# nschejtman/deepLoopCloser

Measured on AMD Instinct MI355X. Metric: query-frames/sec vs N-keyframe DB + top-k recall@1, higher is better.
Workload: dtype bf16; 1 GPU; 1000000 x 4096 bf16 keyframe DB, Q=256, top-20 cosine match, 1 GPU(s); db_rows=1000000, dim=4096, k=20, rows_per_gpu=1000000, pipelined=False, crowded=False

## Files before the change

deeploopcloser_amd/csrc/cosine_topk.hip:

```cpp
#include "dlc_internal.h"

#include <algorithm>

namespace {

constexpr int BM = 256;
constexpr int BNQ = 256;
constexpr int BK = 64;
constexpr int NTHREADS = 512;
constexpr int TILE_BYTES = 256 * BK * 2;
constexpr int A_TILE = TILE_BYTES;
constexpr int B_TILE = TILE_BYTES;
#ifndef DLC_A_STAGES
#define DLC_A_STAGES 2
#endif
constexpr int A_STAGES = DLC_A_STAGES;
constexpr int B_RING = A_STAGES * A_TILE;
constexpr int LDS_BYTES = A_STAGES * A_TILE + 2 * B_TILE;
#ifndef DLC_STAGGER_SLEEP
#define DLC_STAGGER_SLEEP 15
#endif
#ifndef DLC_STAGGER_PHASES
#define DLC_STAGGER_PHASES 32
#endif
// ... 3 lines not shown
constexpr int GROUPS_PER_HALF = HALF / GROUP;
constexpr int SLACK = 4;

template <typename Tag> struct Mfma16;
template <> struct Mfma16<dlc_bf16_tag> {
    static __device__ __forceinline__ f32x4_t run(u32x4_t a, u32x4_t b, f32x4_t c) {
        return __builtin_amdgcn_mfma_f32_16x16x32_bf16(__builtin_bit_cast(bf16x8_t, a),
                                                       __builtin_bit_cast(bf16x8_t, b), c, 0, 0, 0);
    }
    static __device__ __forceinline__ float to_f32(unsigned short h) { return dlc_bf16_bits_to_f32(h); }
};
template <> struct Mfma16<dlc_f16_tag> {
    static __device__ __forceinline__ f32x4_t run(u32x4_t a, u32x4_t b, f32x4_t c) {
        return __builtin_amdgcn_mfma_f32_16x16x32_f16(__builtin_bit_cast(f16x8_t, a),
                                                      __builtin_bit_cast(f16x8_t, b), c, 0, 0, 0);
    }
    static __device__ __forceinline__ float to_f32(unsigned short h) { return dlc_f16_bits_to_f32(h); }
};

typedef const __attribute__((address_space(1))) void* gptr_t;
typedef __attribute__((address_space(3))) void* lptr_t;

__device__ __forceinline__ void glds16(const char* g, char* l) {
    __builtin_amdgcn_global_load_lds((gptr_t)g, (lptr_t)l, 16, 0, 0);
}

__device__ __forceinline__ int swz_a(int r) { return ((r >> 1) & 1) | (((r >> 4) & 3) << 1); }
__device__ __forceinline__ int swz_b(int r) { return (r >> 1) & 7; }

struct GemmArgs {
    const char* Q;
    const char* DB;
    long long ldq_b;
    long long lddb_b;
    int q;
    long long n;
    int nk;
    float* gmax;
    long long ldg;
    float* tmax;
    long long ldt;
    long long ng;
    long long nh;
    float* S;
    long long lds;
    int stagger_mult;
    int stagger_phases;
    int nqb;
    long long ntiles;
    int nsplit;
    int kchunk;
    float* P;
    long long ldp;
};

constexpr int GEMM_GROUPS = 0;
constexpr int GEMM_DENSE = 1;
constexpr int GEMM_PARTIAL = 2;

constexpr int HALF_BYTES = 128 * 128;

#ifndef DLC_A_CACHE_POLICY
#define DLC_A_CACHE_POLICY " nt"
#endif
#define DLC_DMA4_BODY(POLICY)                                \
    asm volatile(                                            \
        "s_nop 4\n\t"                                        \
        "s_mov_b32 %0, m0\n\t"                               \
        "s_mov_b32 m0, %6\n\t"                               \
        "s_nop 0\n\t"                                        \
        "global_load_lds_dwordx4 %1, %5" POLICY "\n\t"       \
        "s_add_u32 m0, %6, 0x400\n\t"                        \
        "s_nop 0\n\t"                                        \
        "global_load_lds_dwordx4 %2, %5" POLICY "\n\t"       \
        "s_add_u32 m0, %6, 0x800\n\t"                        \
        "s_nop 0\n\t"                                        \
        "global_load_lds_dwordx4 %3, %5" POLICY "\n\t"       \
        "s_add_u32 m0, %6, 0xc00\n\t"                        \
        "s_nop 0\n\t"                                        \
        "global_load_lds_dwordx4 %4, %5" POLICY "\n\t"       \
        "s_mov_b32 m0, %0"                                   \
        : "=&s"(keep)                                        \
        : "v"(voff[0]), "v"(voff[1]), "v"(voff[2]), "v"(voff[3]), "s"(sbase), "s"(lds0) \
        : "memory", "scc")
__device__ __forceinline__ void dma4(const unsigned (&voff)[4], const char* sbase, unsigned lds0) {
    unsigned keep;
    DLC_DMA4_BODY("");
}
__device__ __forceinline__ void dma4_stream(const unsigned (&voff)[4], const char* sbase, unsigned lds0) {
    unsigned keep;
    DLC_DMA4_BODY(DLC_A_CACHE_POLICY);
}

#define DLC_WAIT_VMCNT(n) asm volatile("s_waitcnt vmcnt(" #n ")" ::: "memory")
#define DLC_WAIT_LGKM0() asm volatile("s_waitcnt lgkmcnt(0)" ::: "memory")
__device__ __forceinline__ void wg_barrier() {
    asm volatile("" ::: "memory");
    __builtin_amdgcn_s_barrier();
    asm volatile("" ::: "memory");
}

template <typename Tag, int MODE, bool MASKQ>
__global__ __launch_bounds__(NTHREADS, 2) void score_gemm_kernel(GemmArgs p) {
    extern __shared__ __attribute__((aligned(16))) char smem[];
    const int tid = threadIdx.x;
    const int lane = tid & 63;
    const int wid = __builtin_amdgcn_readfirstlane(tid >> 6);
// ... 147 lines not shown
#undef DLC_READ_A
#undef DLC_READ_B
#undef DLC_MFMA
#undef DLC_RELEASE

    const int lg = lane >> 4;
    if constexpr (MODE == GEMM_PARTIAL) {
        float* part = p.P + (long long)chunk * p.q * p.ldp;
#pragma unroll
        for (int c = 0; c < 4; ++c) {
            const int qidx = qblk * BNQ + wc * 64 + c * 16 + i;
            if (qidx >= p.q) continue;
#pragma unroll
            for (int t = 0; t < 8; ++t) {
                const long long row0 = tile * BM + wr * 128 + (t >> 2) * 64 + 16 * lg + 4 * (t & 3);
                *(f32x4_t*)(part + (long long)qidx * p.ldp + row0) = acc[t][c];
            }
        }
    } else if constexpr (MODE == GEMM_DENSE) {
#pragma unroll
        for (int c = 0; c < 4; ++c) {
            const int qidx = qblk * BNQ + wc * 64 + c * 16 + i;
            if (qidx >= p.q) continue;
#pragma unroll
            for (int t = 0; t < 8; ++t) {
                const long long row0 = tile * BM + wr * 128 + (t >> 2) * 64 + 16 * lg + 4 * (t & 3);
#pragma unroll
                for (int r = 0; r < 4; ++r)
                    if (row0 + r < p.n) p.S[(long long)qidx * p.lds + row0 + r] = acc[t][c][r];
            }
        }
    } else {
#pragma unroll
        for (int c = 0; c < 4; ++c) {
            const int qidx = qblk * BNQ + wc * 64 + c * 16 + i;
            float hm[2];
#pragma unroll
            for (int th = 0; th < 2; ++th) {
                float m0 = acc[th * 4][c][0], m1 = acc[th * 4 + 2][c][0];
#pragma unroll
                for (int tt = 0; tt < 2; ++tt)
#pragma unroll
                    for (int r = 0; r < 4; ++r) {
                        m0 = fmaxf(m0, acc[th * 4 + tt][c][r]);
                        m1 = fmaxf(m1, acc[th * 4 + 2 + tt][c][r]);
                    }
                hm[th] = fmaxf(m0, m1);
                const long long g = tile * (BM / GROUP) + wr * 16 + th * 8 + lg * 2;
                if (qidx < p.q) {
                    float* dst = p.gmax + (long long)qidx * p.ldg + g;
                    if (g + 1 < p.ng) *(float2*)dst = make_float2(m0, m1);
                    else if (g < p.ng) dst[0] = m0;
                }
            }
            float h = fmaxf(hm[0], hm[1]);
            h = fmaxf(h, __shfl_xor(h, 16));
            h = fmaxf(h, __shfl_xor(h, 32));
            const long long ht = tile * 2 + wr;
            if (lg == 0 && qidx < p.q && ht < p.nh) p.tmax[(long long)qidx * p.ldt + ht] = h;
        }
    }
}

template <typename Tag> struct Dot2;
template <> struct Dot2<dlc_bf16_tag> {
    typedef __attribute__((ext_vector_type(2))) __bf16 v2_t;
    static __device__ __forceinline__ float run(unsigned a, unsigned b, float c) {
        return __builtin_amdgcn_fdot2_f32_bf16(__builtin_bit_cast(v2_t, a), __builtin_bit_cast(v2_t, b), c, false);
    }
};
template <> struct Dot2<dlc_f16_tag> {
    typedef __attribute__((ext_vector_type(2))) _Float16 v2_t;
    static __device__ __forceinline__ float run(unsigned a, unsigned b, float c) {
        return __builtin_amdgcn_fdot2(__builtin_bit_cast(v2_t, a), __builtin_bit_cast(v2_t, b), c, false);
    }
};

constexpr int GEMV_MAX_Q = 4;
constexpr int GEMV_MAX_LDS = 64 * 1024;

template <typename Tag, int QB>
__global__ __launch_bounds__(256) void score_gemv_kernel(GemmArgs p) {
    extern __shared__ __attribute__((aligned(16))) char smem[];
    __shared__ float wmax[4][QB];
    const int tid = threadIdx.x, lane = tid & 63, w = tid >> 6;
    const long long half = blockIdx.x;
    const int d_bytes = p.nk * 128;
    for (int off = tid * 16; off < QB * d_bytes; off += 256 * 16) {
        const int qi = off / d_bytes, within = off - qi * d_bytes;
        uint4 v = make_uint4(0, 0, 0, 0);
        if (qi < p.q) v = *(const uint4*)(p.Q + (long long)qi * p.ldq_b + within);
        *(uint4*)(smem + off) = v;
    }
    __syncthreads();
    float hmax[QB];
#pragma unroll
    for (int qq = 0; qq < QB; ++qq) hmax[qq] = -INFINITY;
    for (int gi = 0; gi < 4; ++gi) {
        const long long g = half * GROUPS_PER_HALF + w * 4 + gi;
        const char* rows[GROUP];
#pragma unroll
        for (int r = 0; r < GROUP; ++r) {
            long long rr = g * GROUP + r;
            if (rr > p.n - 1) rr = p.n - 1;
            rows[r] = p.DB + rr * p.lddb_b;
        }
// ... 28 lines not shown
                float v = acc[qq][r];
#pragma unroll
                for (int o = 32; o > 0; o >>= 1) v += __shfl_xor(v, o);
                m = fmaxf(m, v);
            }
            hmax[qq] = fmaxf(hmax[qq], m);
            if (lane == 0 && qq < p.q && g < p.ng) p.gmax[(long long)qq * p.ldg + g] = m;
        }
    }
    if (lane == 0) {
#pragma unroll
        for (int qq = 0; qq < QB; ++qq) wmax[w][qq] = hmax[qq];
    }
    __syncthreads();
    if (tid < QB && tid < p.q && half < p.nh)
        p.tmax[(long long)tid * p.ldt + half] = fmaxf(fmaxf(wmax[0][tid], wmax[1][tid]), fmaxf(wmax[2][tid], wmax[3][tid]));
}

__device__ __forceinline__ unsigned f32_key(float x) {
    unsigned u = __float_as_uint(x);
    return (u & 0x80000000u) ? ~u : (u | 0x80000000u);
}
__device__ __forceinline__ float key_f32(unsigned k) {
    return __uint_as_float((k & 0x80000000u) ? (k ^ 0x80000000u) : ~k);
}
__device__ __forceinline__ unsigned long long pack_key(float score, unsigned id) {
    return ((unsigned long long)f32_key(score) << 32) | (unsigned long long)(~id);
}
__device__ __forceinline__ unsigned key_id(unsigned long long key) { return ~(unsigned)key; }

constexpr long long KEY64_EMPTY = (long long)0x8000000000000000ull;
__device__ __forceinline__ long long f64_key(double s) {
    const double x = s * 1099511627776.0;
    if (!(x > -4.0e18)) return KEY64_EMPTY + 1;
    if (x > 4.0e18) return 0x7fffffffffffffffll;
    return __double2ll_rn(x);
}

__device__ __forceinline__ unsigned wave_max_u32(unsigned v) {
#define DLC_DPP_MAX(ctrl, rmask) \
    v = max(v, (unsigned)__builtin_amdgcn_update_dpp((int)v, (int)v, ctrl, rmask, 0xf, false))
    DLC_DPP_MAX(0x111, 0xf);
    DLC_DPP_MAX(0x112, 0xf);
    DLC_DPP_MAX(0x114, 0xf);
    DLC_DPP_MAX(0x118, 0xf);
    DLC_DPP_MAX(0x142, 0xa);
    DLC_DPP_MAX(0x143, 0xc);
#undef DLC_DPP_MAX
    return (unsigned)__builtin_amdgcn_readlane((int)v, 63);
}

constexpr int FIN_THREADS = 512;
__host__ __device__ inline size_t fin_lds_fixed(int kg) {
    return (size_t)kg * (GROUPS_PER_HALF * 8 + GROUP * (8 + 8 + 4)) + (size_t)(kg + 1) * 8 + 64;
}

__device__ __forceinline__ void rank_select(const unsigned long long* keys, int m, int k, int* out, bool plus_one = false) {
    const int lim = plus_one ? k + 1 : k;
    for (int e = threadIdx.x; e < m; e += blockDim.x) {
        const unsigned long long ke = keys[e];
        if (ke == 0ull) continue;
        int rank = 0;
#pragma unroll 8
        for (int j = 0; j < m; ++j) rank += keys[j] > ke ? 1 : 0;
        if (rank < lim) out[rank] = e;
    }
}
template <typename Id>
__device__ __forceinline__ void rank_select64(const long long* keys, const Id* ids, int m, int k, int* out) {
    for (int e = threadIdx.x; e < m; e += blockDim.x) {
        const long long ke = keys[e];
        if (ke == KEY64_EMPTY) continue;
        const Id ie = ids[e];
        int rank = 0;
#pragma unroll 4
        for (int j = 0; j < m; ++j) {
            const long long kj = keys[j];
            rank += (kj > ke || (kj == ke && kj != KEY64_EMPTY && ids[j] < ie)) ? 1 : 0;
        }
        if (rank < k) out[rank] = e;
    }
}

template <typename Tag, int RS_UNROLL>
__device__ __forceinline__ void rescore8_f64(const char* qrow, const char* const (&rows)[GROUP], int d, int lane,
                                             double (&acc)[GROUP]) {
#pragma unroll
    for (int r = 0; r < GROUP; ++r) acc[r] = 0.0;
    for (int d0 = lane * 8; d0 < d; d0 += 512 * RS_UNROLL) {
        uint4 qv[RS_UNROLL], rv[RS_UNROLL][GROUP];
#pragma unroll
        for (int u = 0; u < RS_UNROLL; ++u) {
            const int dd = d0 + u * 512;
            const bool ok = dd < d;
            qv[u] = ok ? *(const uint4*)(qrow + (long long)dd * 2) : make_uint4(0, 0, 0, 0);
#pragma unroll
            for (int r = 0; r < GROUP; ++r)
                rv[u][r] = ok ? *(const uint4*)(rows[r] + (long long)dd * 2) : make_uint4(0, 0, 0, 0);
        }
#pragma unroll
        for (int u = 0; u < RS_UNROLL; ++u) {
            const unsigned qw[4] = {qv[u].x, qv[u].y, qv[u].z, qv[u].w};
            double qd[8];
#pragma unroll
            for (int e = 0; e < 4; ++e) {
                qd[2 * e] = (double)Mfma16<Tag>::to_f32((unsigned short)(qw[e] & 0xffffu));
                qd[2 * e + 1] = (double)Mfma16<Tag>::to_f32((unsigned short)(qw[e] >> 16));
// ... 48 lines not shown
#pragma unroll
                for (int e = 0; e < 4; ++e) {
                    acc[r] = fma(qd[2 * e], (double)Mfma16<Tag>::to_f32((unsigned short)(w4[e] & 0xffffu)), acc[r]);
                    acc[r] = fma(qd[2 * e + 1], (double)Mfma16<Tag>::to_f32((unsigned short)(w4[e] >> 16)), acc[r]);
                }
            }
        }
    }
#pragma unroll
    for (int r = 0; r < R; ++r) {
        double v = acc[r];
#pragma unroll
        for (int o = 32; o > 0; o >>= 1) v += __shfl_xor(v, o);
        acc[r] = v;
    }
}
template <typename Tag>
__device__ __forceinline__ double rescore1_f64(const char* qrow, const char* row, int d, int lane) {
    const char* const rows[1] = {row};
    double acc[1];
    rescore_rows_f64<Tag, 1, 4>(qrow, rows, d, lane, acc);
    return acc[0];
}

__device__ __forceinline__ double scaled_tau(double tau, const float* __restrict__ tau_scale, int qi) {
    return tau_scale ? tau * (double)tau_scale[qi] : tau;
}

enum { FIN_FUSED = 0, FIN_GROUPS = 1, FIN_RESCORE = 2 };
struct FinishArgs {
    float* tmax; long long ldt; int nh; int tv_in_lds;
    const float* gmax; long long ldg; long long ng;
    int kg;
    const char* Q; long long ldq_b; const char* DB; long long lddb_b;
    long long n; int d; int k; long long row_offset;
    float* out_s;
    double* out_s64;
    long long* out_i;
    int* status;
    double tau;
    const float* tau_scale;
    int* grp_ids;
    float* grp_max;
    const float* all_max;
    int parts;
    long long nq;
    int gparts;
    float* bound_out;
    const float* dense_S;
    long long ld_s;
    int rslack;
    int limited;
    long long limit0;
};
__device__ __forceinline__ long long visible_rows(long long n, int limited, long long limit0, int qi) {
    if (!limited) return n;
    const long long lim = limit0 + qi;
    return lim < 0 ? 0 : (lim < n ? lim : n);
}

template <typename Tag, int THREADS, int RS_UNROLL, int MODE>
__device__ __forceinline__ void finish_topk_body(const FinishArgs& a) {
    extern __shared__ __attribute__((aligned(16))) char dsm[];
    constexpr int FIN_WAVES = THREADS / 64;
    constexpr int FIN_THREADS = THREADS;
    constexpr int GPH = GROUPS_PER_HALF;
    const int kg = a.kg, k = a.k;
    const double tau = scaled_tau(a.tau, a.tau_scale, (int)blockIdx.x);
    const long long n = visible_rows(a.n, a.limited, a.limit0, (int)blockIdx.x);
    const long long ng = a.limited ? (n + GROUP - 1) / GROUP : a.ng;
    if (n <= 0) {
        if constexpr (MODE == FIN_GROUPS) {
            for (int e = threadIdx.x; e <= kg; e += THREADS) {
                if (e < kg) a.grp_ids[(long long)blockIdx.x * kg + e] = -1;
                a.grp_max[(long long)blockIdx.x * (kg + 1) + e] = -INFINITY;
            }
        } else {
            const long long oq = (long long)blockIdx.y * a.nq + blockIdx.x;
            for (int e = threadIdx.x; e < k; e += THREADS) {
                if (a.out_s) a.out_s[oq * k + e] = -INFINITY;
                a.out_s64[oq * k + e] = -INFINITY;
                a.out_i[oq * k + e] = -1;
            }
            if (MODE == FIN_FUSED && threadIdx.x == 0) a.status[blockIdx.x] = 0;
            if (MODE == FIN_RESCORE && a.bound_out && blockIdx.y == 0 && threadIdx.x == 0) a.bound_out[blockIdx.x] = -INFINITY;
        }
        return;
    }
    unsigned long long* ckey = (unsigned long long*)dsm;
    long long* ck64 = (long long*)(dsm + (size_t)kg * GPH * 8);
    double* cs64 = (double*)(dsm + (size_t)kg * (GPH * 8 + GROUP * 8));
    int* crow = (int*)(dsm + (size_t)kg * (GPH * 8 + GROUP * 16));
    int* sel = (int*)(dsm + (size_t)kg * (GPH * 8 + GROUP * 20));
    int* sel2 = sel + kg + 1;
    unsigned* misc = (unsigned*)(sel2 + kg + 1);
    const int qi = blockIdx.x, tid = threadIdx.x, lane = tid & 63, w = tid >> 6;
    float* tv = a.tv_in_lds ? (float*)(dsm + fin_lds_fixed(kg)) : a.tmax + (long long)qi * a.ldt;
    if (a.tv_in_lds)
        for (int e = tid; e < a.nh; e += FIN_THREADS) tv[e] = a.tmax[(long long)qi * a.ldt + e];
    for (int e = tid; e <= kg; e += FIN_THREADS) { sel[e] = -1; sel2[e] = -1; }
    if (tid < 16) misc[tid] = 0u;
    __syncthreads();
    int kg2;
    unsigned bkey = 0u;
    if constexpr (MODE != FIN_RESCORE) {
    const int nh = a.limited ? (int)((n + HALF - 1) / HALF) : a.nh;
    const int kt = min(kg, nh);
    {
        const int chunk = (nh + FIN_WAVES - 1) / FIN_WAVES;
        const int lo_e = w * chunk, hi_e = min(nh, lo_e + chunk);
        unsigned bh = 0, bl = 0;
        constexpr int LV = 16;
        if ((THREADS == 512 || MODE == FIN_GROUPS) && chunk <= 64 * LV) {
            unsigned vk[LV];
#pragma unroll
            for (int j = 0; j < LV; ++j) {
                const int e = lo_e + lane + 64 * j;
                const float v = e < hi_e ? tv[e] : -INFINITY;
                vk[j] = v == -INFINITY ? 0u : f32_key(v);
            }
            auto rescan_regs = [&]() {
                bh = 0; bl = 0;
#pragma unroll
                for (int j = 0; j < LV; ++j) {
                    const unsigned l = ~(unsigned)(lo_e + lane + 64 * j);
                    if (vk[j] > bh) { bh = vk[j]; bl = l; }
                }
            };
            rescan_regs();
            for (int it = 0; it < kt; ++it) {
                const unsigned mh = wave_max_u32(bh);
                const unsigned ml = wave_max_u32(bh == mh ? bl : 0u);
                if (lane == 0) ckey[w * kt + it] = mh == 0u ? 0ull : (((unsigned long long)mh << 32) | ml);
                if (mh != 0u && bh == mh && bl == ml) {
                    const int jr = (int)((~ml) - (unsigned)(lo_e + lane)) >> 6;
#pragma unroll
                    for (int j = 0; j < LV; ++j)
                        if (j == jr) vk[j] = 0u;
                    rescan_regs();
                }
            }
        } else {
        auto rescan = [&]() {
            bh = 0; bl = 0;
            for (int e = lo_e + lane; e < hi_e; e += 64) {
                const float v = tv[e];
                if (v == -INFINITY) continue;
                const unsigned h = f32_key(v), l = ~(unsigned)e;
                if (h > bh || (h == bh && l > bl)) { bh = h; bl = l; }
            }
        };
        rescan();
        for (int it = 0; it < kt; ++it) {
            const unsigned mh = wave_max_u32(bh);
            const unsigned ml = wave_max_u32(bh == mh ? bl : 0u);
            if (lane == 0) ckey[w * kt + it] = mh == 0u ? 0ull : (((unsigned long long)mh << 32) | ml);
            if (mh != 0u && bh == mh && bl == ml) {
                tv[~ml] = -INFINITY;
                rescan();
            }
        }
        }
        const unsigned rest = wave_max_u32(bh);
        if (lane == 0) misc[w] = rest;
    }
    __syncthreads();
    rank_select(ckey, FIN_WAVES * kt, kt, sel, true);
    __syncthreads();
#pragma unroll
    for (int ww = 0; ww < FIN_WAVES; ++ww) bkey = max(bkey, misc[ww]);
    if (sel[kt] >= 0) bkey = max(bkey, (unsigned)(ckey[sel[kt]] >> 32));
    if (tid < kt) { const int c = sel[tid]; sel[tid] = c < 0 ? -1 : (int)key_id(ckey[c]); }
    __syncthreads();

    const int m2 = kt * GPH;
    for (int e = tid; e < m2; e += FIN_THREADS) {
        const int ht = sel[e / GPH];
        const long long g = (long long)ht * GPH + (e % GPH);
        float gm = (ht >= 0 && g < ng) ? a.gmax[(long long)qi * a.ldg + g] : 0.0f;
        if (a.limited && a.dense_S && ht >= 0 && g == ng - 1 && (n & (GROUP - 1))) {
            gm = -INFINITY;
            for (long long row = g * GROUP; row < n; ++row) gm = fmaxf(gm, a.dense_S[(long long)qi * a.ld_s + row]);
        }
        ckey[e] = (ht >= 0 && g < ng) ? pack_key(gm, (unsigned)g) : 0ull;
    }
    __syncthreads();
    kg2 = min(kg, m2);
    rank_select(ckey, m2, kg2, sel2, true);
    __syncthreads();
    if (sel2[kg2] >= 0) bkey = max(bkey, (unsigned)(ckey[sel2[kg2]] >> 32));
    if constexpr (MODE == FIN_GROUPS) {
        const long long W = kg + 1;
        for (int e = tid; e < kg; e += FIN_THREADS) {
            const int c = e < kg2 ? sel2[e] : -1;
            a.grp_ids[(long long)qi * kg + e] = c < 0 ? -1 : (int)key_id(ckey[c]);
            a.grp_max[(long long)qi * W + e] = c < 0 ? -INFINITY : a.gmax[(long long)qi * a.ldg + key_id(ckey[c])];
        }
        if (tid == 0) a.grp_max[(long long)qi * W + kg] = bkey ? key_f32(bkey) : -INFINITY;
        return;
    }
    if (tid < kg2) {
        const int c = sel2[tid];
        int g = c < 0 ? -1 : (int)key_id(ckey[c]);
        if (tid >= k && g >= 0 && sel2[k - 1] >= 0 && !(a.limited && !a.dense_S)) {
            const double uk = (double)key_f32((unsigned)(ckey[sel2[k - 1]] >> 32));
            if ((double)key_f32((unsigned)(ckey[c] >> 32)) < uk - 2.0 * tau) g = -2;
        }
        misc[9] = 0u;
        crow[tid] = g;
    }
    __syncthreads();
    if (tid < kg2) {
        const int g = crow[tid];
        if (g == -2) atomicMax(&misc[9], (unsigned)(ckey[sel2[tid]] >> 32));
    }
    __syncthreads();
    if (tid < kg2) sel2[tid] = crow[tid] < 0 ? -1 : crow[tid];
    bkey = max(bkey, misc[9]);
    __syncthreads();
    } else {
        kg2 = kg;
        const long long W = kg + 1;
        if (a.parts > 0) {
            unsigned bk = 0u;
            for (int e = tid; e < a.parts * (int)W; e += FIN_THREADS) {
                const int pp = e / (int)W, j = e % (int)W;
                const float v = a.all_max[((long long)pp * a.nq + qi) * W + j];
                if (v == -INFINITY) continue;
                if (j == kg) { bk = max(bk, f32_key(v)); continue; }
                int greater = 0;
                for (int p2 = 0; p2 < a.parts; ++p2) {
                    const float* av = a.all_max + ((long long)p2 * a.nq + qi) * W;
                    for (int j2 = 0; j2 < kg; ++j2) greater += av[j2] > v ? 1 : 0;
                }
                if (greater >= kg) bk = max(bk, f32_key(v));
            }
            if (bk) atomicMax(&misc[8], bk);
        }
        for (int e = tid; e < kg; e += FIN_THREADS) {
            int g = a.grp_ids[(long long)qi * kg + e];
            if (g >= 0 && a.parts > 0) {
                const float v = a.grp_max[(long long)qi * W + e];
                int greater = 0;
                for (int pp = 0; pp < a.parts; ++pp) {
                    const float* av = a.all_max + ((long long)pp * a.nq + qi) * W;
                    for (int j = 0; j < kg; ++j) greater += av[j] > v ? 1 : 0;
                }
                if (greater >= kg) g = -1;
            }
            if (a.gparts > 1 && e % a.gparts != (int)blockIdx.y) g = -1;
            sel2[e] = g;
        }
        __syncthreads();
        if (a.parts > 0) bkey = misc[8];
        else {
            const float v = a.grp_max[(long long)qi * W + kg];
            bkey = v == -INFINITY ? 0u : f32_key(v);
        }
        if (a.bound_out && blockIdx.y == 0 && tid == 0) a.bound_out[qi] = bkey ? key_f32(bkey) : -INFINITY;
    }

    int m3;
    if (a.dense_S) {
        const int m = kg2 * GROUP;
        for (int e = tid; e < m; e += FIN_THREADS) {
            const int g = sel2[e / GROUP];
            const long long row = (long long)g * GROUP + (e % GROUP);
            ckey[e] = (g >= 0 && row < n) ? pack_key(a.dense_S[(long long)qi * a.ld_s + row], (unsigned)row) : 0ull;
        }
        m3 = min(k + a.rslack, m);
        for (int e = tid; e <= m3 && e < kg * GROUP; e += FIN_THREADS) crow[e] = -1;
        __syncthreads();
        if (m3 < m) rank_select(ckey, m, m3, crow, true);
        else rank_select(ckey, m, m3, crow, false);
        __syncthreads();
        if (m3 < m && crow[m3] >= 0) bkey = max(bkey, (unsigned)(ckey[crow[m3]] >> 32));
        __syncthreads();
        for (int e = tid; e < m3; e += FIN_THREADS) { const int c = crow[e]; crow[e] = c < 0 ? -1 : (int)key_id(ckey[c]); }
    } else {
        m3 = kg2 * GROUP;
        for (int e = tid; e < m3; e += FIN_THREADS) {
            const int g = sel2[e / GROUP];
            const long long row = (long long)g * GROUP + (e % GROUP);
            crow[e] = (g >= 0 && row < n) ? (int)row : -1;
        }
    }
    __syncthreads();

    const char* qrow = a.Q + (long long)qi * a.ldq_b;
    if (MODE == FIN_FUSED && a.dense_S != nullptr) {
        for (int ci = w; ci < m3; ci += FIN_WAVES) {
            const int id = __builtin_amdgcn_readfirstlane(crow[ci]);
            const double sc = id < 0 ? 0.0 : rescore1_f64<Tag>(qrow, a.DB + (long long)id * a.lddb_b, a.d, lane);
            if (lane == 0) {
                cs64[ci] = id < 0 ? -INFINITY : sc;
                ck64[ci] = id < 0 ? KEY64_EMPTY : f64_key(sc);
            }
        }
    } else
    for (int s = w; s * GROUP < m3; s += FIN_WAVES) {
        int ids[GROUP];
        bool any = false;
        const char* rows[GROUP];
#pragma unroll
        for (int r = 0; r < GROUP; ++r) {
            ids[r] = __builtin_amdgcn_readfirstlane(s * GROUP + r < m3 ? crow[s * GROUP + r] : -1);
            any |= ids[r] >= 0;
            rows[r] = a.DB + (long long)(ids[r] < 0 ? 0 : ids[r]) * a.lddb_b;
        }
        double acc[GROUP] = {0.0, 0.0, 0.0, 0.0, 0.0, 0.0, 0.0, 0.0};
        if (any) rescore8_f64<Tag, RS_UNROLL>(qrow, rows, a.d, lane, acc);
#pragma unroll
        for (int r = 0; r < GROUP; ++r)
            if (lane == r && s * GROUP + r < m3) {
                cs64[s * GROUP + r] = ids[r] < 0 ? -INFINITY : acc[r];
                ck64[s * GROUP + r] = ids[r] < 0 ? KEY64_EMPTY : f64_key(acc[r]);
            }
    }
    const long long oq = (long long)blockIdx.y * a.nq + qi;
    for (int e = tid; e < k; e += FIN_THREADS) {
        if (a.out_s) a.out_s[oq * k + e] = -INFINITY;
        a.out_s64[oq * k + e] = -INFINITY;
        a.out_i[oq * k + e] = -1;
    }
    for (int e = tid; e <= kg; e += FIN_THREADS) sel[e] = -1;
    __syncthreads();

    rank_select64(ck64, crow, m3, k, sel);
    __syncthreads();
    for (int e = tid; e < k; e += FIN_THREADS) {
        const int c = sel[e];
        if (c >= 0) {
            if (a.out_s) a.out_s[oq * k + e] = (float)cs64[c];
            a.out_s64[oq * k + e] = cs64[c];
            a.out_i[oq * k + e] = (long long)crow[c] + a.row_offset;
        }
    }
    if constexpr (MODE == FIN_FUSED) {
        if (tid == 0) {
            const int c = sel[k - 1];
            const bool cert = bkey == 0u || (c >= 0 && cs64[c] > (double)key_f32(bkey) + tau);
            a.status[qi] = cert ? 0 : 1;
        }
    }
}

template <typename Tag, int THREADS, int RS_UNROLL, int MODE>
__global__ __launch_bounds__(THREADS) void finish_topk_kernel(FinishArgs a) {
    finish_topk_body<Tag, THREADS, RS_UNROLL, MODE>(a);
}
template <typename Tag, int RS_UNROLL, int MODE>
__global__ __launch_bounds__(256) __attribute__((amdgpu_waves_per_eu(5))) void finish_topk_coop_kernel(FinishArgs a) {
    finish_topk_body<Tag, 256, RS_UNROLL, MODE>(a);
}

struct ExhaustiveArgs {
    const float* gmax; long long ldg; long long ng;
    const char* Q; long long ldq_b; const char* DB; long long lddb_b;
    long long n; int d; int k; long long row_offset;
    const double* lower; long long lower_stride;
    float* out_s; double* out_s64; long long* out_i;
    int* status;
    double tau;
    const float* tau_scale;
    int limited; long long limit0;
};
constexpr int EXH_BATCH = 64;
constexpr int EXH_POOL = EXH_BATCH * GROUP + DLC_MAX_K;

template <typename Tag, int RS_UNROLL = 4>
// ... 492 lines not shown
    m = fmaxf(m, __shfl_xor(m, 1));
    m = fmaxf(m, __shfl_xor(m, 2));
    m = fmaxf(m, __shfl_xor(m, 4));
    m = fmaxf(m, __shfl_xor(m, 8));
    const long long ht = g / GROUPS_PER_HALF;
    if ((threadIdx.x & 15) == 0 && ht < nh) tmax[(long long)qi * ldt + ht] = m;
}

__global__ __launch_bounds__(256) void splitk_dense_kernel(const float* __restrict__ P, long long ldp, int q, int nsplit,
                                                           float* __restrict__ S, long long lds, long long n) {
    const int qi = blockIdx.x;
    const long long r0 = ((long long)blockIdx.y * 256 + threadIdx.x) * 4;
    if (r0 >= n) return;
    f64x4_t a64 = {0., 0., 0., 0.};
    const float* src = P + (long long)qi * ldp + r0;
    for (int c = 0; c < nsplit; ++c) {
        a64 += __builtin_convertvector(*(const f32x4_t*)src, f64x4_t);
        src += (long long)q * ldp;
    }
    const f32x4_t a = __builtin_convertvector(a64, f32x4_t);
#pragma unroll
    for (int r = 0; r < 4; ++r)
        if (r0 + r < n) S[(long long)qi * lds + r0 + r] = a[r];
}

struct SplitPlan {
    int nsplit, kchunk;
};
SplitPlan split_plan(int64_t q, int64_t n, int64_t d) {
    const int64_t ntiles = dlc::cdiv(n, BM);
    const int64_t base = dlc::cdiv(ntiles, (int64_t)8) * 8 * dlc::cdiv(q, BNQ);
    const int64_t nk = d / BK;
    SplitPlan best{1, (int)nk};
    if (base >= 256 || nk < 8) return best;
    const double t_k = 1.6, t_fix = 8.0, t_launch = 5.0, bytes_per_us = 3.0e6;
    const double part_bytes = (double)q * (double)ntiles * BM * 4.0;
    const int64_t work = ntiles * dlc::cdiv(q, BNQ);
    double best_t = (double)dlc::cdiv(work, (int64_t)256) * ((double)nk * t_k + t_fix);
    for (int64_t ns = 2; ns <= nk / 4 && ns <= 256; ++ns) {
        const int64_t kc = dlc::cdiv(nk, ns), ns_eff = dlc::cdiv(nk, kc);
        if (ns_eff != ns) continue;
        if ((double)ns_eff * part_bytes > (double)(1ll << 30)) break;
        const double t = (double)dlc::cdiv(work * ns_eff, (int64_t)256) * ((double)kc * t_k + t_fix) +
                         2.0 * (double)ns_eff * part_bytes / bytes_per_us + t_launch;
        if (t < best_t * 0.9) {
            best_t = t;
            best = SplitPlan{(int)ns_eff, (int)kc};
        }
    }
    return best;
}

struct WsLayout {
    size_t gmax, tmax, part, status, s64, rs_ids, rs_max, rs_scores, rs_idx, rs_bound, total;
    long long ldg, ldt, ldp;
    int kg;
    SplitPlan sp;
    int rparts;
    bool dense;
    double tau;
};

inline bool gemv_shape(int64_t q, int64_t nk) {
    const int qb = q <= 1 ? 1 : (q <= 2 ? 2 : 4);
    return q <= GEMV_MAX_Q && (long long)qb * nk * 128 <= GEMV_MAX_LDS;
}

constexpr int64_t DENSE_MAX_ROWS = 16384;
constexpr int DENSE_ROW_SLACK = 4;
constexpr int64_t DENSE_GEMV_BYTES = 32ll << 20;
inline bool dense_plan(int64_t q, int64_t n, int64_t d) {
    return n <= DENSE_MAX_ROWS && (!gemv_shape(q, d / BK) || n * d * 2 <= DENSE_GEMV_BYTES);
}

int rescore_parts(int64_t q, int64_t d, int kg, int k) {
    if (q > 32 || (int64_t)kg * GROUP * d * 2 < (2 << 20)) return 1;
    return std::min(kg, 2048 / k);
}

constexpr double SCORE_STEP_EPS = 1.1920928955078125e-07;
double score_error_bound(int64_t q, int64_t nk, const SplitPlan& sp, bool dense) {
    double steps;
    if (!dense && gemv_shape(q, nk)) steps = (double)nk * 0.5 + 8.0;
    else steps = 2.0 * (double)sp.kchunk + 2.0;
    return SCORE_STEP_EPS * 1.01 * steps + 3.7e-12;
}

WsLayout ws_layout(int64_t q, int64_t n, int64_t d, int k) {
    WsLayout w;
    const int64_t ntiles = dlc::cdiv(n, BM);
    w.ldg = ntiles * (BM / GROUP);
    w.ldt = ntiles * 2;
    w.kg = k + SLACK;
    size_t o = 0;
    w.gmax = o; o += dlc::align_up((size_t)q * w.ldg * 4, 256);
    w.tmax = o; o += dlc::align_up((size_t)q * w.ldt * 4, 256);
    w.sp = split_plan(q, n, d);
    w.dense = dense_plan(q, n, d);
    w.tau = score_error_bound(q, d / BK, w.sp, w.dense);
    w.ldp = ntiles * BM;
    w.part = o;
    if (w.sp.nsplit > 1 || w.dense) o += dlc::align_up((size_t)w.sp.nsplit * q * w.ldp * 4, 256);
    w.status = o; o += dlc::align_up((size_t)q * 4, 256);
    w.s64 = o; o += dlc::align_up((size_t)q * k * 8, 256);
    w.rparts = w.dense ? 1 : rescore_parts(q, d, w.kg, k);
    w.rs_ids = w.rs_max = w.rs_scores = w.rs_idx = w.rs_bound = o;
    if (w.rparts > 1) {
        w.rs_ids = o; o += dlc::align_up((size_t)q * w.kg * 4, 256);
        w.rs_max = o; o += dlc::align_up((size_t)q * (w.kg + 1) * 4, 256);
        w.rs_scores = o; o += dlc::align_up((size_t)w.rparts * q * k * 8, 256);
        w.rs_idx = o; o += dlc::align_up((size_t)w.rparts * q * k * 8, 256);
        w.rs_bound = o; o += dlc::align_up((size_t)q * 4, 256);
    }
    w.total = o;
    return w;
}

int check_operands(dlc_ctx* ctx, int dtype, const void* Q, int64_t q, int64_t ldq, const void* DB, int64_t n,
                   int64_t lddb, int64_t d) {
    if (!ctx) return DLC_ERR_BAD_ARG;
    if (dtype != DLC_BF16 && dtype != DLC_F16)
        return dlc::fail(ctx, DLC_ERR_UNSUPPORTED, "cosine match: dtype %d (need DLC_BF16 or DLC_F16)", dtype);
    if (!Q || !DB || q < 1 || n < 1 || d < 1) return dlc::fail(ctx, DLC_ERR_BAD_ARG, "cosine match: null/empty operand");
    if (d % BK != 0) return dlc::fail(ctx, DLC_ERR_BAD_SHAPE, "cosine match: d=%lld must be a multiple of %d", (long long)d, BK);
    if (ldq < d || lddb < d || (ldq % 8) || (lddb % 8))
        return dlc::fail(ctx, DLC_ERR_BAD_SHAPE, "cosine match: row strides must be >= d and multiples of 8 elements");
    if (((uintptr_t)Q & 15) || ((uintptr_t)DB & 15))
        return dlc::fail(ctx, DLC_ERR_BAD_ARG, "cosine match: operands must be 16-byte aligned");
    if (ldq * 2 * 255 + 128 > 0xffffffffll || lddb * 2 * 255 + 128 > 0xffffffffll)
        return dlc::fail(ctx, DLC_ERR_BAD_SHAPE, "cosine match: row stride %lld elements too large (255 rows must span < 4 GiB)",
                         (long long)(ldq > lddb ? ldq : lddb));
    if (q > 0x7fffff00ll) return dlc::fail(ctx, DLC_ERR_BAD_SHAPE, "cosine match: q too large");
    if (n > 0x7ffffff0ll) return dlc::fail(ctx, DLC_ERR_BAD_SHAPE, "cosine match: more than 2^31 rows in one shard");
    return DLC_OK;
}

template <typename Tag, int MODE, bool MASKQ>
int launch_gemm_masked(dlc_ctx* ctx, const GemmArgs& a, hipStream_t st);

template <typename Tag, int MODE>
int launch_gemm(dlc_ctx* ctx, const GemmArgs& a, hipStream_t st) {
    const int tail = a.q % BNQ;
    return (tail > 0 && tail <= 192) ? launch_gemm_masked<Tag, MODE, true>(ctx, a, st)
                                     : launch_gemm_masked<Tag, MODE, false>(ctx, a, st);
}

template <typename Tag> constexpr int tag_id() { return __is_same(Tag, dlc_bf16_tag) ? 0 : 1; }

template <typename K>
int raise_lds_limit(dlc_ctx* ctx, K kern, int bit, int bytes) {
    const unsigned long long m = 1ull << bit;
    if (!(ctx->func_attr_set & m)) {
        DLC_HIP_CHECK(ctx, hipFuncSetAttribute((const void*)kern, hipFuncAttributeMaxDynamicSharedMemorySize, bytes));
        ctx->func_attr_set |= m;
    }
    return DLC_OK;
}

template <typename Tag, int MODE, bool MASKQ>
int launch_gemm_masked(dlc_ctx* ctx, const GemmArgs& a, hipStream_t st) {
    auto kern = score_gemm_kernel<Tag, MODE, MASKQ>;
    int rc_attr = raise_lds_limit(ctx, kern, DLC_ATTR_GEMM_BASE + tag_id<Tag>() * 8 + MODE * 2 + (MASKQ ? 1 : 0), LDS_BYTES);
    if (rc_attr != DLC_OK) return rc_attr;
    GemmArgs b = a;
    b.ntiles = dlc::cdiv(a.n, BM);
    b.nqb = (int)dlc::cdiv(a.q, BNQ);
// ... 34 lines not shown
    if (a.nsplit <= 1 && !keep)
        return dense ? launch_gemm<Tag, GEMM_DENSE>(ctx, a, st) : launch_gemm<Tag, GEMM_GROUPS>(ctx, a, st);
    int rc = launch_gemm<Tag, GEMM_PARTIAL>(ctx, a, st);
    if (rc != DLC_OK) return rc;
    if (partials_only) return DLC_OK;
    if (dense) {
        dim3 grid((unsigned)a.q, (unsigned)dlc::cdiv(a.n, (int64_t)1024));
        hipLaunchKernelGGL(splitk_dense_kernel, grid, dim3(256), 0, st, a.P, a.ldp, a.q, a.nsplit, a.S, a.lds, a.n);
        DLC_LAUNCH_CHECK(ctx, "splitk_dense_kernel");
    } else {
        const long long groups = dlc::cdiv(a.n, BM) * (BM / GROUP);
        dim3 grid((unsigned)a.q, (unsigned)dlc::cdiv(groups, (long long)256));
        hipLaunchKernelGGL(splitk_groups_kernel, grid, dim3(256), 0, st, a.P, a.ldp, a.q, a.nsplit, a.gmax, a.ldg, a.ng,
                           a.tmax, a.ldt, a.nh, keep ? 1 : 0);
        DLC_LAUNCH_CHECK(ctx, "splitk_groups_kernel");
    }
    return DLC_OK;
}

}

extern "C" size_t dlc_cosine_topk_workspace_bytes(int64_t q, int64_t n, int64_t d, int k) {
    if (q < 1 || n < 1 || d < BK || k < 1 || k > DLC_MAX_K) return 0;
    return ws_layout(q, n, d, k).total;
}

namespace {

struct MatchCall {
    GemmArgs a;
    WsLayout w;
};

int prepare_match(dlc_ctx* ctx, const char* what, int dtype, const void* Q, int64_t q, int64_t ldq, const void* DB,
                  int64_t n, int64_t lddb, int64_t d, int k, void* workspace, size_t workspace_bytes, MatchCall* mc) {
    int rc = check_operands(ctx, dtype, Q, q, ldq, DB, n, lddb, d);
    if (rc != DLC_OK) return rc;
    if (k < 1 || k > DLC_MAX_K) return dlc::fail(ctx, DLC_ERR_BAD_ARG, "%s: k=%d outside 1..%d", what, k, DLC_MAX_K);
    mc->w = ws_layout(q, n, d, k);
    if (!workspace || workspace_bytes < mc->w.total)
        return dlc::fail(ctx, DLC_ERR_WORKSPACE, "%s: workspace %zu < %zu bytes", what, workspace_bytes, mc->w.total);
    if (((uintptr_t)workspace & 255)) return dlc::fail(ctx, DLC_ERR_BAD_ARG, "%s: workspace must be 256-byte aligned", what);
    char* ws = (char*)workspace;
    GemmArgs& a = mc->a;
    a.Q = (const char*)Q; a.DB = (const char*)DB;
    a.ldq_b = ldq * 2; a.lddb_b = lddb * 2;
    a.q = (int)q; a.n = n; a.nk = (int)(d / BK);
    a.gmax = (float*)(ws + mc->w.gmax); a.ldg = mc->w.ldg;
    a.tmax = (float*)(ws + mc->w.tmax); a.ldt = mc->w.ldt;
    a.ng = dlc::cdiv(n, GROUP); a.nh = dlc::cdiv(n, HALF);
    a.S = nullptr; a.lds = 0;
    a.nsplit = mc->w.sp.nsplit; a.kchunk = mc->w.sp.kchunk;
    a.P = (float*)(ws + mc->w.part); a.ldp = mc->w.ldp;
    return DLC_OK;
}

inline bool small_direct(const MatchCall& mc, int k) {
    return mc.w.dense && mc.a.n <= (int64_t)FIN_THREADS * SMALL_GPT * GROUP && k + DENSE_ROW_SLACK + 1 <= SMALL_KT_MAX;
}

int run_score(dlc_ctx* ctx, int dtype, MatchCall& mc, hipStream_t st, bool partials_only = false) {
    return dlc::profiled(ctx, st, [&]() -> int {
        return (dtype == DLC_BF16) ? launch_scores<dlc_bf16_tag>(ctx, mc.a, false, st, mc.w.dense, partials_only)
                                   : launch_scores<dlc_f16_tag>(ctx, mc.a, false, st, mc.w.dense, partials_only);
    });
}

FinishArgs finish_args(const MatchCall& mc, int k, int64_t n, int64_t d, int64_t q, int64_t row_offset) {
    const GemmArgs& g = mc.a;
    FinishArgs f{};
    f.tmax = g.tmax; f.ldt = g.ldt; f.nh = (int)g.nh;
    f.gmax = g.gmax; f.ldg = g.ldg; f.ng = g.ng;
    f.kg = mc.w.kg;
    f.Q = g.Q; f.ldq_b = g.ldq_b; f.DB = g.DB; f.lddb_b = g.lddb_b;
    f.n = n; f.d = (int)d; f.k = k; f.row_offset = row_offset;
    f.tau = mc.w.tau;
    f.nq = q;
    return f;
}

template <typename Tag, int THREADS, int RS_UNROLL, int MODE>
int launch_finish(dlc_ctx* ctx, FinishArgs f, int64_t q, bool small_lds, hipStream_t st) {
    size_t dsm = fin_lds_fixed(f.kg);
    f.tv_in_lds = MODE != FIN_RESCORE && !small_lds && (size_t)f.nh * 4 <= 96 * 1024;
    if (f.tv_in_lds) dsm += (size_t)f.nh * 4;
    dsm = dlc::align_up(dsm, 16);
    void (*fk)(FinishArgs);
    if constexpr (THREADS == 256) fk = finish_topk_coop_kernel<Tag, RS_UNROLL, MODE>;
    else fk = finish_topk_kernel<Tag, THREADS, RS_UNROLL, MODE>;
    if (dsm > 48 * 1024)
        DLC_HIP_CHECK(ctx, hipFuncSetAttribute((const void*)fk, hipFuncAttributeMaxDynamicSharedMemorySize, (int)dsm));
    hipLaunchKernelGGL(fk, dim3((unsigned)q, (unsigned)(MODE == FIN_RESCORE && f.gparts > 1 ? f.gparts : 1)), dim3(THREADS),
                       dsm, st, f);
    DLC_LAUNCH_CHECK(ctx, "finish_topk_kernel");
    return DLC_OK;
}

template <int MODE>
int run_select(dlc_ctx* ctx, int dtype, const FinishArgs& f, int64_t q, int flags, hipStream_t st) {
    const bool coop = (flags & DLC_SELECT_COOP) != 0;
    if (dtype == DLC_BF16)
        return coop ? launch_finish<dlc_bf16_tag, 256, 1, MODE>(ctx, f, q, true, st)
                    : launch_finish<dlc_bf16_tag, 512, 4, MODE>(ctx, f, q, false, st);
    return coop ? launch_finish<dlc_f16_tag, 256, 1, MODE>(ctx, f, q, true, st)
                : launch_finish<dlc_f16_tag, 512, 4, MODE>(ctx, f, q, false, st);
}

int run_exhaustive(dlc_ctx* ctx, int dtype, const FinishArgs& f, int64_t q, const double* lower, int64_t lower_stride,
                   float* out_s, double* out_s64, int64_t* out_i, int* status, hipStream_t st) {
    ExhaustiveArgs e{};
    e.gmax = f.gmax; e.ldg = f.ldg; e.ng = f.ng;
    e.Q = f.Q; e.ldq_b = f.ldq_b; e.DB = f.DB; e.lddb_b = f.lddb_b;
    e.n = f.n; e.d = f.d; e.k = f.k; e.row_offset = f.row_offset;
    e.lower = lower; e.lower_stride = lower_stride;
    e.out_s = out_s; e.out_s64 = out_s64; e.out_i = (long long*)out_i;
    e.status = status; e.tau = f.tau; e.tau_scale = f.tau_scale;
    e.limited = f.limited; e.limit0 = f.limit0;
    if (dtype == DLC_BF16)
        hipLaunchKernelGGL(exhaustive_topk_kernel<dlc_bf16_tag>, dim3((unsigned)q), dim3(FIN_THREADS), 0, st, e);
    else
        hipLaunchKernelGGL(exhaustive_topk_kernel<dlc_f16_tag>, dim3((unsigned)q), dim3(FIN_THREADS), 0, st, e);
    DLC_LAUNCH_CHECK(ctx, "exhaustive_topk_kernel");
    return DLC_OK;
}

int launch_merge(dlc_ctx* ctx, const double* scores, int64_t score_part_stride, const int64_t* idx, int64_t idx_part_stride,
                 int parts, int64_t q, int k, const float* bound, double tau, const float* tau_scale, float* out_scores,
                 double* out_scores_f64, int64_t* out_idx, int* status, hipStream_t st) {
    const size_t m = (size_t)parts * k;
    const size_t dsm = m * 24;
// ... 434 lines not shown
```

Measured before the change: 124,300 query-frames/s.

## Record per-group argmax and runner-up bound to rescore single rows instead of full groups

The GEMM epilogue now writes a 16-bit record per 8-row group holding the index of its maximum row and a quantized upper bound on its runner-up score. The fused finish kernel reads these records and, when a candidate group's runner-up cannot reach the k-th bound minus 2·tau, rescores only that group's best row in fp64 rather than all eight rows. It also folds the skipped runner-up bound into the reported threshold. This aims to cut the fp64 rescoring DB reads in the finish stage. The cost is extra epilogue ALU work, an additional q×ng ushort workspace write and read, and more LDS in the finish kernel.

```diff
diff --git a/deeploopcloser_amd/csrc/cosine_topk.hip b/deeploopcloser_amd/csrc/cosine_topk.hip
--- a/deeploopcloser_amd/csrc/cosine_topk.hip
+++ b/deeploopcloser_amd/csrc/cosine_topk.hip
@@ -79,7 +79,31 @@
     int kchunk;
     float* P;
     long long ldp;
+    unsigned short* grec;
 };
+
+__device__ __forceinline__ unsigned group_record(const float (&v)[8]) {
+    float h[4], l[4];
+    unsigned ix[4];
+#pragma unroll
+    for (int p = 0; p < 4; ++p) {
+        const bool rt = v[2 * p + 1] > v[2 * p];
+        h[p] = rt ? v[2 * p + 1] : v[2 * p];
+        l[p] = rt ? v[2 * p] : v[2 * p + 1];
+        ix[p] = rt ? 2u * p + 1u : 2u * p;
+    }
+    const bool r0 = h[1] > h[0], r1 = h[3] > h[2];
+    const float h0 = r0 ? h[1] : h[0], l0 = r0 ? h[0] : h[1];
+    const float h1 = r1 ? h[3] : h[2], l1 = r1 ? h[2] : h[3];
+    const unsigned i0 = r0 ? ix[1] : ix[0], i1 = r1 ? ix[3] : ix[2];
+    const bool r2 = h1 > h0;
+    const unsigned idx = r2 ? i1 : i0;
+    const float ru = fmaxf(fmaxf(fmaxf(l[0], l[1]), fmaxf(l[2], l[3])), fmaxf(fmaxf(l0, l1), r2 ? h0 : h1));
+    const unsigned u = __float_as_uint(ru);
+    const unsigned key = (u & 0x80000000u) ? ~u : (u | 0x80000000u);
+    const unsigned code = __builtin_elementwise_add_sat(key, 0x7ffffu) >> 19;
+    return (code << 3) | idx;
+}
 
 constexpr int GEMM_GROUPS = 0;
 constexpr int GEMM_DENSE = 1;
@@ -333,6 +357,20 @@
                     if (g + 1 < p.ng) *(float2*)dst = make_float2(m0, m1);
                     else if (g < p.ng) dst[0] = m0;
                 }
+                if (p.grec && qidx < p.q) {
+                    float v0[8], v1[8];
+#pragma unroll
+                    for (int tt = 0; tt < 2; ++tt)
+#pragma unroll
+                        for (int r = 0; r < 4; ++r) {
+                            v0[4 * tt + r] = acc[th * 4 + tt][c][r];
+                            v1[4 * tt + r] = acc[th * 4 + 2 + tt][c][r];
+                        }
+                    const unsigned r0 = group_record(v0), r1 = group_record(v1);
+                    unsigned short* rd = p.grec + (long long)qidx * p.ldg + g;
+                    if (g + 1 < p.ng) *(unsigned*)rd = r0 | (r1 << 16);
+                    else if (g < p.ng) rd[0] = (unsigned short)r0;
+                }
             }
             float h = fmaxf(hm[0], hm[1]);
             h = fmaxf(h, __shfl_xor(h, 16));
@@ -467,7 +505,7 @@
 
 constexpr int FIN_THREADS = 512;
 __host__ __device__ inline size_t fin_lds_fixed(int kg) {
-    return (size_t)kg * (GROUPS_PER_HALF * 8 + GROUP * (8 + 8 + 4)) + (size_t)(kg + 1) * 8 + 64;
+    return (size_t)kg * (GROUPS_PER_HALF * 8 + GROUP * (8 + 8 + 4) + GROUPS_PER_HALF * 2) + (size_t)(kg + 1) * 8 + 64;
 }
 
 __device__ __forceinline__ void rank_select(const unsigned long long* keys, int m, int k, int* out, bool plus_one = false) {
@@ -622,6 +660,7 @@
     int rslack;
     int limited;
     long long limit0;
+    const unsigned short* grec;
 };
 __device__ __forceinline__ long long visible_rows(long long n, int limited, long long limit0, int qi) {
     if (!limited) return n;
@@ -664,6 +703,7 @@
     int* sel = (int*)(dsm + (size_t)kg * (GPH * 8 + GROUP * 20));
     int* sel2 = sel + kg + 1;
     unsigned* misc = (unsigned*)(sel2 + kg + 1);
+    unsigned short* crec = (unsigned short*)(misc + 16);
     const int qi = blockIdx.x, tid = threadIdx.x, lane = tid & 63, w = tid >> 6;
     float* tv = a.tv_in_lds ? (float*)(dsm + fin_lds_fixed(kg)) : a.tmax + (long long)qi * a.ldt;
     if (a.tv_in_lds)
@@ -753,6 +793,7 @@
             for (long long row = g * GROUP; row < n; ++row) gm = fmaxf(gm, a.dense_S[(long long)qi * a.ld_s + row]);
         }
         ckey[e] = (ht >= 0 && g < ng) ? pack_key(gm, (unsigned)g) : 0ull;
+        if (MODE == FIN_FUSED && a.grec) crec[e] = (ht >= 0 && g < ng) ? a.grec[(long long)qi * a.ldg + g] : (unsigned short)0xffffu;
     }
     __syncthreads();
     kg2 = min(kg, m2);
@@ -772,17 +813,24 @@
     if (tid < kg2) {
         const int c = sel2[tid];
         int g = c < 0 ? -1 : (int)key_id(ckey[c]);
-        if (tid >= k && g >= 0 && sel2[k - 1] >= 0 && !(a.limited && !a.dense_S)) {
+        int r1 = -1;
+        if (g >= 0 && sel2[k - 1] >= 0 && !(a.limited && !a.dense_S)) {
             const double uk = (double)key_f32((unsigned)(ckey[sel2[k - 1]] >> 32));
-            if ((double)key_f32((unsigned)(ckey[c] >> 32)) < uk - 2.0 * tau) g = -2;
+            if (tid >= k && (double)key_f32((unsigned)(ckey[c] >> 32)) < uk - 2.0 * tau) g = -2;
+            if (MODE == FIN_FUSED && a.grec && g >= 0) {
+                const unsigned rec = crec[c];
+                if ((double)key_f32((rec >> 3) << 19) < uk - 2.0 * tau) r1 = g * GROUP + (int)(rec & 7u);
+            }
         }
         misc[9] = 0u;
         crow[tid] = g;
+        sel[tid] = r1;
     }
     __syncthreads();
     if (tid < kg2) {
         const int g = crow[tid];
         if (g == -2) atomicMax(&misc[9], (unsigned)(ckey[sel2[tid]] >> 32));
+        if (sel[tid] >= 0) atomicMax(&misc[9], ((unsigned)crec[sel2[tid]] >> 3) << 19);
     }
     __syncthreads();
     if (tid < kg2) sel2[tid] = crow[tid] < 0 ? -1 : crow[tid];
@@ -830,7 +878,7 @@
         if (a.bound_out && blockIdx.y == 0 && tid == 0) a.bound_out[qi] = bkey ? key_f32(bkey) : -INFINITY;
     }
 
-    int m3;
+    int m3, nfull = 0;
     if (a.dense_S) {
         const int m = kg2 * GROUP;
         for (int e = tid; e < m; e += FIN_THREADS) {
@@ -848,12 +896,25 @@
         __syncthreads();
         for (int e = tid; e < m3; e += FIN_THREADS) { const int c = crow[e]; crow[e] = c < 0 ? -1 : (int)key_id(ckey[c]); }
     } else {
-        m3 = kg2 * GROUP;
-        for (int e = tid; e < m3; e += FIN_THREADS) {
-            const int g = sel2[e / GROUP];
-            const long long row = (long long)g * GROUP + (e % GROUP);
-            crow[e] = (g >= 0 && row < n) ? (int)row : -1;
-        }
+        int* rstash = (int*)ckey;
+        if (tid < kg2 && sel2[tid] >= 0) {
+            const int g = sel2[tid], r1 = MODE == FIN_FUSED ? sel[tid] : -1;
+            if (r1 < 0) {
+                const int s = (int)atomicAdd(&misc[11], 1u);
+#pragma unroll
+                for (int r = 0; r < GROUP; ++r) {
+                    const long long row = (long long)g * GROUP + r;
+                    crow[s * GROUP + r] = row < n ? (int)row : -1;
+                }
+            } else {
+                rstash[atomicAdd(&misc[12], 1u)] = r1;
+            }
+        }
+        __syncthreads();
+        nfull = (int)misc[11];
+        const int nrows = (int)misc[12];
+        m3 = nfull * GROUP + nrows;
+        for (int e = tid; e < nrows; e += FIN_THREADS) crow[nfull * GROUP + e] = rstash[e];
     }
     __syncthreads();
 
@@ -867,14 +928,14 @@
                 ck64[ci] = id < 0 ? KEY64_EMPTY : f64_key(sc);
             }
         }
-    } else
-    for (int s = w; s * GROUP < m3; s += FIN_WAVES) {
+    } else {
+    for (int s = w; s < nfull; s += FIN_WAVES) {
         int ids[GROUP];
         bool any = false;
         const char* rows[GROUP];
 #pragma unroll
         for (int r = 0; r < GROUP; ++r) {
-            ids[r] = __builtin_amdgcn_readfirstlane(s * GROUP + r < m3 ? crow[s * GROUP + r] : -1);
+            ids[r] = __builtin_amdgcn_readfirstlane(crow[s * GROUP + r]);
             any |= ids[r] >= 0;
             rows[r] = a.DB + (long long)(ids[r] < 0 ? 0 : ids[r]) * a.lddb_b;
         }
@@ -882,10 +943,34 @@
         if (any) rescore8_f64<Tag, RS_UNROLL>(qrow, rows, a.d, lane, acc);
 #pragma unroll
         for (int r = 0; r < GROUP; ++r)
-            if (lane == r && s * GROUP + r < m3) {
+            if (lane == r) {
                 cs64[s * GROUP + r] = ids[r] < 0 ? -INFINITY : acc[r];
                 ck64[s * GROUP + r] = ids[r] < 0 ? KEY64_EMPTY : f64_key(acc[r]);
             }
+    }
+    const int base = nfull * GROUP, nrows = m3 - base;
+    int ci = (w + FIN_WAVES - nfull % FIN_WAVES) % FIN_WAVES;
+    for (; ci + FIN_WAVES < nrows; ci += 2 * FIN_WAVES) {
+        const int id0 = __builtin_amdgcn_readfirstlane(crow[base + ci]);
+        const int id1 = __builtin_amdgcn_readfirstlane(crow[base + ci + FIN_WAVES]);
+        const char* const rows[2] = {a.DB + (long long)id0 * a.lddb_b, a.DB + (long long)id1 * a.lddb_b};
+        double sc[2];
+        rescore_rows_f64<Tag, 2, 4>(qrow, rows, a.d, lane, sc);
+        if (lane == 0) {
+            cs64[base + ci] = sc[0];
+            ck64[base + ci] = f64_key(sc[0]);
+            cs64[base + ci + FIN_WAVES] = sc[1];
+            ck64[base + ci + FIN_WAVES] = f64_key(sc[1]);
+        }
+    }
+    if (ci < nrows) {
+        const int id = __builtin_amdgcn_readfirstlane(crow[base + ci]);
+        const double sc = rescore1_f64<Tag>(qrow, a.DB + (long long)id * a.lddb_b, a.d, lane);
+        if (lane == 0) {
+            cs64[base + ci] = sc;
+            ck64[base + ci] = f64_key(sc);
+        }
+    }
     }
     const long long oq = (long long)blockIdx.y * a.nq + qi;
     for (int e = tid; e < k; e += FIN_THREADS) {
@@ -1484,12 +1569,13 @@
 }
 
 struct WsLayout {
-    size_t gmax, tmax, part, status, s64, rs_ids, rs_max, rs_scores, rs_idx, rs_bound, total;
+    size_t gmax, tmax, part, status, s64, rs_ids, rs_max, rs_scores, rs_idx, rs_bound, grec, total;
     long long ldg, ldt, ldp;
     int kg;
     SplitPlan sp;
     int rparts;
     bool dense;
+    bool rec;
     double tau;
 };
 
@@ -1544,6 +1630,9 @@
         w.rs_idx = o; o += dlc::align_up((size_t)w.rparts * q * k * 8, 256);
         w.rs_bound = o; o += dlc::align_up((size_t)q * 4, 256);
     }
+    w.rec = !w.dense && w.sp.nsplit <= 1 && !gemv_shape(q, d / BK);
+    w.grec = o;
+    if (w.rec) o += dlc::align_up((size_t)q * w.ldg * 2, 256);
     w.total = o;
     return w;
 }
@@ -1684,6 +1773,7 @@
     a.S = nullptr; a.lds = 0;
     a.nsplit = mc->w.sp.nsplit; a.kchunk = mc->w.sp.kchunk;
     a.P = (float*)(ws + mc->w.part); a.ldp = mc->w.ldp;
+    a.grec = mc->w.rec ? (unsigned short*)(ws + mc->w.grec) : nullptr;
     return DLC_OK;
 }
 
@@ -1708,6 +1798,7 @@
     f.n = n; f.d = (int)d; f.k = k; f.row_offset = row_offset;
     f.tau = mc.w.tau;
     f.nq = q;
+    f.grec = g.grec;
     return f;
 }
 
```

Measured after the change: 124,600 query-frames/s (median of 6 runs). About the same (+0.3%).
